# microsoft/fadtk

Measured on AMD Instinct MI355X. Metric: FAD scores/sec + cov-GEMM TFLOP/s (% MFMA peak), N=100k D=512, higher is better.
Workload: dtype f16 in, f16 MFMA with f32 accumulate over <= 8192-row runs, f64 across runs (moments); split-f16 MFMA iterations (f32 accumulate) + exact int8-MFMA products (int32 accumulate) + f64 correction (Frechet)

## Files before the change

fadtk_amd/csrc/frechet.hip:

```cpp
#include "frechet_internal.h"
#include "ns_mean.h"
#include "ns_fast.h"
#include "ns_fast_big.h"
#include "ns_fast_res.h"

#include <algorithm>
#include <atomic>
#include <cmath>
#include <type_traits>

namespace fad {

Pool& thread_pool(int device) {
    static thread_local PerThreadDevice<Pool> set;
    return set.get(device);
}
Workspace* free_slot(int device) {
    Pool& p = thread_pool(device);
    for (Workspace& w : p.slot)
        if (!w.busy) { w.pool = &p; return &w; }
    return nullptr;
}

SongKnobs SongKnobs::from_env() {
// ... 359 lines not shown
        g.k = k; g.max_low = max_low; g.nslots = nslots; g.chk_partials = m.partials;
        g.thr_pred = pred_threshold(ws.pool, d);
        fast_split(d, nsf::SP_U, g, stream, 1);
    }
    nsf::I8Args a;
    memset(&a, 0, sizeof(a));
    a.Adig = f.digY[0]; a.Bdig = f.digYt[0]; a.Adig_alt = f.digY[1]; a.Bdig_alt = f.digYt[1]; a.sel = &m.s32->final_iter;
    a.d = d; a.gen = ws.job.gen; a.hA = f.hdr; a.hB = f.hdr + 1; a.skip = &m.s32->skip_corr; a.stats = f.host_stats; a.st = m.dstate; a.A64in = m.A;
    a.Y[0] = f.Y[0]; a.Y[1] = f.Y[1]; a.Z[0] = f.Z[0]; a.Z[1] = f.Z[1];
    a.s32 = m.s32; a.host_words = f.host_words; a.host_vals = f.host_vals;
    const bool wide = wide_enabled(ws.pool);
    if (wide) { a.Rv = f.Rv; a.scaled = 1; }
    f.host_words[12] = 0;
    f.host_words[13] = 0;
    fast_i8(d, nsf::I8_G, a, stream);
    FAD_HIP_TRY(hipGetLastError());
    if (!ws.done_ev) FAD_HIP_TRY(hipEventCreateWithFlags(&ws.done_ev, hipEventDisableTiming));
    if (wide && ws.pool && ws.pool->lp_verify) return fast_verify_enqueue(ws);
    FAD_HIP_TRY(hipEventRecord(ws.done_ev, stream));
    return FAD_OK;
}

static void fast_decide_one(const int* hw, const double* hv, const double* hsx, int nb, MixedResult* out, const double* hvx = nullptr,
                            int gen = 0, int max_low = kMaxLow) {
    MixedResult o;
    memset(&o, 0, sizeof(o));
    const bool bad = hw[0] != 0;
    o.status = 0; o.iters = hw[7]; o.decided_at = hw[8]; o.nonfinite = hw[2]; o.too_few0 = hw[3]; o.too_few1 = hw[4];
    o.c = hv[0]; o.tr1 = hv[1]; o.tr2 = hv[2]; o.mean_term = hv[3];
    o.prepared = 0;
    const bool ok = hw[5] != 0, failed = hw[6] != 0, strict = hw[9] != 0;
    if (bad || hw[1] || failed) {
        o.status = 2;
    } else if (ok && !hw[11]) {
        double corr = 0.0, r2 = 0.0, tr = 0.0, zinf = 0.0, zone = 0.0;
        for (int t = 0; t < nb * nb; ++t) { corr += hsx[nsf::kTileStats * t]; r2 += hsx[nsf::kTileStats * t + 1]; tr += hsx[nsf::kTileStats * t + 2]; }
        const double* zmax = hsx + (size_t)nsf::kTileStats * nb * nb;
        for (int x = 0; x < nb; ++x) {
            double rs = 0.0, cs = 0.0;
            for (int y = 0; y < nb; ++y) { rs += zmax[2 * (y * nb + x)]; cs += zmax[2 * (x * nb + y) + 1]; }
            if (rs > zinf) zinf = rs;
            if (cs > zone) zone = cs;
        }
        const int fi = hw[7];
        double res = hv[4 + ns32_slot(fi)];
        if (hw[8] == fi - 1) { const double rp = hv[4 + ns32_slot(fi - 1)]; res = 0.75 * rp * rp + 0.25 * rp * rp * rp; if (res < 2e-6) res = 2e-6; }
        const double zn = std::sqrt(zinf * zone), rn = std::sqrt(r2);
        double trs = tr + 0.5 * corr;
        double est = zn * zn * zn * rn * rn / 8.0 + zn * res * rn / 2.0;
        bool finite = std::isfinite(trs) && std::isfinite(est);
        double fad = o.mean_term + o.tr1 + o.tr2 - 2.0 * std::sqrt(o.c) * trs;
        bool accept = finite && (est <= 1e-9 * std::fabs(trs) || 2.0 * std::sqrt(o.c) * est <= 1e-5 * std::fabs(fad));
        const bool scaled = hvx && hw[14] != 0;
        const bool predicted = hw[8] == fi - 1 && fi >= 1;
        const double r_pred = predicted ? hv[4 + ns32_slot(fi - 1)] : 0.0;
        const bool can_go_on = predicted && !strict && fi + 1 < max_low && (!scaled || r_pred > 0.1);
        bool need_verify = false;
        if (!accept && finite && hvx && !can_go_on) {
            if (hw[13] == gen) {
                const double inv = 1.0 / ((double)nsf::kVerScale * (double)nsf::kVerScale);
                double qp = 0.0, ep = 0.0, pp = 0.0, ee = 0.0;
// ... 34 lines not shown

bool fast_song_dim(int d) { return d == 128 || d == 256 || d == 384 || d == 512 || d == 768 || d == 1024; }

struct SongBlock {
    size_t hdr, st, s32, partials, stats, A64, P, Y[2], Z[2], T, digS, digY[2], digYt[2], stride;
};
static SongBlock song_block(int d) {
    const size_t dd = (size_t)d * d, nb = (size_t)d / 32;
    SongBlock b; size_t o = 0;
    auto take = [&](size_t bytes) { const size_t at = o; o += (bytes + 255) & ~(size_t)255; return at; };
    b.hdr = take(sizeof(nsf::MatHdr)); b.st = take(sizeof(NsState)); b.s32 = take(sizeof(Ns32State));
    b.partials = take(nb * nb * sizeof(double)); b.stats = take(nsf::kTileStats * nb * nb * sizeof(double));
    b.A64 = take(8 * dd); b.P = take(8 * dd);
    b.Y[0] = take(8 * dd); b.Y[1] = take(8 * dd); b.Z[0] = take(8 * dd); b.Z[1] = take(8 * dd); b.T = take(8 * dd);
    b.digS = take(6 * dd);
    b.digY[0] = take(6 * dd); b.digYt[0] = take(6 * dd); b.digY[1] = take(6 * dd); b.digYt[1] = take(6 * dd);
    b.stride = o;
    return b;
}
static size_t host_vstats_off(int d) {
    const size_t nb = (size_t)d / 32;
    return (nsf::kHostVals + (nsf::kTileStats + 2) * nb * nb) * sizeof(double) + ((nsf::kHostWords * sizeof(int) + 7) & ~(size_t)7);
}
static size_t song_host_stride(int d) {
    const size_t nb = (size_t)d / 32;
    return (host_vstats_off(d) + nsf::kVerStats * nb * nb * sizeof(double) + 63) & ~(size_t)63;
}
int64_t fast_songs_capacity(int d, size_t budget_bytes) {
    const int64_t n = (int64_t)(budget_bytes / song_block(d).stride);
    return n < 1 ? 1 : (n > 16384 ? 16384 : n);
}

int fast_songs(int d, int64_t B, const double* dcov_b, const double* covs, hipStream_t st, Workspace& ws,
               std::vector<double>& tr_sqrt, std::vector<char>& ok, int device, const SongKnobs& knobs) {
    const bool big = knobs.big_min > 0 && B >= knobs.big_min;
    const bool resident = d == 128 && knobs.res != 0;
    const bool res_full = resident && knobs.res != 1;
    const bool scaled_steps = knobs.scaled && big && d >= 256;
    const bool scaled_res = knobs.scaled && resident;
    const size_t dd = (size_t)d * d;
    const int nb = d / 32;
    const SongBlock L = song_block(d);
    const size_t hs = song_host_stride(d);
    FAD_TRY(ws.fast_songs.reserve(512 + 6 * dd + (size_t)B * L.stride));
    if (!ws.fast_songs_pin || ws.fast_songs_pin_cap < (size_t)B * hs) {
        if (ws.fast_songs_pin) (void)hipHostFree(ws.fast_songs_pin);
        ws.fast_songs_pin = nullptr; ws.fast_songs_pin_cap = 0;
        FAD_HIP_TRY(hipHostMalloc(&ws.fast_songs_pin, (size_t)B * hs + 4096, hipHostMallocDefault));
        ws.fast_songs_pin_cap = (size_t)B * hs + 4096;
    }
// ... 120 lines not shown
            if (hw[12] != gen) return set_error(FAD_ERR_HIP, "the correction kernel of the batched fast chain left no result for song %lld", (long long)b);
            MixedResult r;
            fast_decide_one(hw, hv, hx, nb, &r);
            if (r.status == 0 && k < kMaxLow && !resident) { pending = true; continue; }
            settled[b] = 1;
            if (r.status == 1) { ok[b] = 1; tr_sqrt[b] = std::sqrt(r.c) * r.tr_scaled; }
            if (trace)
                fprintf(stderr, "[fad fast songs] song %lld: status %d iters %d decided_at %d res %.3e est %.3e tr %.6e c %.3e (words bad %d done %d ok %d failed %d skipped %d)\n",
                        (long long)b, r.status, r.iters, r.decided_at, r.res, r.est, r.tr_scaled, r.c, hw[0], hw[1], hw[5], hw[6], hw[11]);
            if (trace && b == 0) {
                fprintf(stderr, "[fad fast songs] song 0 residuals:");
                for (int q = 1; q < 16 && q <= r.iters; ++q) fprintf(stderr, " %.3e", hv[4 + q]);
                fprintf(stderr, "\n");
            }
        }
        if (!pending) break;
        upto = kMaxLow;
    }
    return FAD_OK;
}


struct PairBlock {
    size_t hdrA, hdrB, st, s32, partials, stats, A64, P, Y[2], Z[2], T, digA, digB, digY[2], digYt[2], mus, covs, Rv, Pv, Ev, stride;
};
static PairBlock pair_block(int d) {
    const size_t dd = (size_t)d * d, nb = (size_t)d / 32;
    PairBlock b; size_t o = 0;
    auto take = [&](size_t bytes) { const size_t at = o; o += (bytes + 255) & ~(size_t)255; return at; };
    b.hdrA = take(sizeof(nsf::MatHdr)); b.hdrB = take(sizeof(nsf::MatHdr)); b.st = take(sizeof(NsState)); b.s32 = take(sizeof(Ns32State));
    b.partials = take(nb * nb * sizeof(double)); b.stats = take(nsf::kTileStats * nb * nb * sizeof(double));
    b.A64 = take(8 * dd); b.P = take(8 * dd);
    b.Y[0] = take(8 * dd); b.Y[1] = take(8 * dd); b.Z[0] = take(8 * dd); b.Z[1] = take(8 * dd); b.T = take(8 * dd);
    b.digA = take(6 * dd); b.digB = take(6 * dd);
    b.digY[0] = take(6 * dd); b.digYt[0] = take(6 * dd); b.digY[1] = take(6 * dd); b.digYt[1] = take(6 * dd);
    b.mus = take(2 * (size_t)d * sizeof(double)); b.covs = take(2 * dd * sizeof(double));
    b.Rv = take(8 * dd); b.Pv = take(8 * dd); b.Ev = take(8 * dd);
    b.stride = o;
    return b;
}

static int pairs_verify_enqueue(Workspace& ws, int d, int B, hipStream_t st) {
    const size_t dd = (size_t)d * d;
    const PairBlock L = pair_block(d);
    const size_t hs = song_host_stride(d);
    char* blk = static_cast<char*>(ws.fast_pairs.p);
    char* hpin = static_cast<char*>(ws.fast_pairs_pin);
    auto at = [&](size_t off) { return blk + off; };
    auto mat = [&](size_t off) { nsf::SplitMat m; m.a = reinterpret_cast<uint4*>(at(off)); m.at = reinterpret_cast<uint4*>(at(off + 4 * dd)); return m; };
    nsf::SplitArgs g;
    memset(&g, 0, sizeof(g));
    g.d = d; g.gen = ws.multi.gen; g.hA = reinterpret_cast<nsf::MatHdr*>(at(L.hdrA)); g.hB = reinterpret_cast<nsf::MatHdr*>(at(L.hdrB));
    g.pstride = (int64_t)L.stride; g.astride = (int64_t)L.stride;
    g.st = reinterpret_cast<NsState*>(at(L.st)); g.s32 = reinterpret_cast<Ns32State*>(at(L.s32));
    const nsf::SplitMat Y[2] = {mat(L.Y[0]), mat(L.Y[1])}, Z[2] = {mat(L.Z[0]), mat(L.Z[1])};
    const int nb = d / 32;
    int* h_words = reinterpret_cast<int*>(hpin + (nsf::kHostVals + (size_t)(nsf::kTileStats + 2) * nb * nb) * sizeof(double));
    double* h_vstats = reinterpret_cast<double*>(hpin + host_vstats_off(d));
    for (int b = 0; b < B; ++b) reinterpret_cast<int*>(reinterpret_cast<char*>(h_words) + (size_t)b * hs)[13] = 0;
    fast_verify_launch(d, (unsigned)B, g, Y, Z, mat(L.Rv), mat(L.Pv), mat(L.Ev), g.s32, h_vstats, h_words, (int64_t)hs, st);
    FAD_HIP_TRY(hipGetLastError());
    FAD_HIP_TRY(hipEventRecord(ws.done_ev, st));
    return FAD_OK;
}

static int pairs_enqueue(Workspace& ws, int d, int B, const fad_moments_t* const* h1, const fad_moments_t* const* h2, int ddof,
                         int mean_dtype, hipStream_t st) {
    const size_t dd = (size_t)d * d;
    const int nb = d / 32;
    constexpr int kPairsBigMin = 3;
    const bool big = B >= kPairsBigMin && d >= 256;
    const bool wide = wide_enabled(ws.pool);
    const int max_low = wide ? kMaxLowWide : kMaxLow;
    const int device = ws.job.device;
    const PairBlock L = pair_block(d);
    const size_t hs = song_host_stride(d);
    void* const before = ws.fast_pairs.p;
    FAD_TRY(ws.fast_pairs.reserve((size_t)(B > 16 ? kMaxMultiPairs : B > 8 ? 16 : B > 4 ? 8 : 4) * L.stride + 256));
    if (!ws.fast_pairs_pin || ws.fast_pairs_pin_cap < (size_t)B * hs) {
        if (ws.fast_pairs_pin) (void)hipHostFree(ws.fast_pairs_pin);
        ws.fast_pairs_pin = nullptr; ws.fast_pairs_pin_cap = 0;
        FAD_HIP_TRY(hipHostMalloc(&ws.fast_pairs_pin, (size_t)kMaxMultiPairs * hs + 4096, hipHostMallocDefault));
        ws.fast_pairs_pin_cap = (size_t)kMaxMultiPairs * hs + 4096;
    }
    char* blk = static_cast<char*>(ws.fast_pairs.p);
    char* hpin = static_cast<char*>(ws.fast_pairs_pin);
    double* h_vals = reinterpret_cast<double*>(hpin);
    double* h_stats = h_vals + nsf::kHostVals;
    int* h_words = reinterpret_cast<int*>(h_stats + (size_t)(nsf::kTileStats + 2) * nb * nb);
    auto at = [&](size_t off) { return blk + off; };
    auto mat = [&](size_t off) { nsf::SplitMat m; m.a = reinterpret_cast<uint4*>(at(off)); m.at = reinterpret_cast<uint4*>(at(off + 4 * dd)); return m; };
    const int gen = ++ws.fast_gen;
    if (ws.fast_gen > (1 << 30)) ws.fast_gen = 1;
    ws.multi.gen = gen;
// ... 21 lines not shown
    }
    pa.acc[0] = pa.accs[0]; pa.acc[1] = pa.accs[1];
    pa.d = d; pa.ddof = ddof; pa.gen = gen; pa.mean_dtype = mean_dtype;
    pa.mus = reinterpret_cast<double*>(at(L.mus)); pa.covs = reinterpret_cast<double*>(at(L.covs));
    pa.dig[0] = reinterpret_cast<uint4*>(at(L.digA)); pa.dig[1] = reinterpret_cast<uint4*>(at(L.digB));
    pa.st = st0; pa.hdr[0] = hA; pa.hdr[1] = hB;
    pa.batch = 2; pa.pstride = (int64_t)L.stride; pa.no_covs = 1;
    pa.per = ((dd / 2048) % 4 == 0) ? 4 : 2;
    hipLaunchKernelGGL(nsf::nsf_prepare, dim3((unsigned)(dd / 2048 / pa.per + 1), (unsigned)(2 * B)), dim3(512), 0, st, pa);

    auto split_args = [&]() {
        nsf::SplitArgs g;
        memset(&g, 0, sizeof(g));
        g.d = d; g.gen = gen; g.hA = hA; g.hB = hB; g.pstride = (int64_t)L.stride; g.astride = (int64_t)L.stride;
        g.st = st0; g.s32 = s32_0;
        if (wide) { g.scaled = 1; g.lp_wide = 1; g.l0_scale = kWideL0Scale; g.l0_min = kWideL0Min; }
        return g;
    };
    {
        nsf::I8Args a;
        memset(&a, 0, sizeof(a));
        a.Adig = reinterpret_cast<uint4*>(at(L.digA)); a.Bdig = reinterpret_cast<uint4*>(at(L.digB)); a.d = d; a.gen = gen; a.hA = hA; a.hB = hB;
        a.pstride = (int64_t)L.stride; a.astride = (int64_t)L.stride; a.stats = stats; a.A64 = A64; a.P = P; a.st = st0;
        if (big) FAD_TRY(fast_i8_big(d, nsf::I8_A, a, st, (unsigned)B, device));
        else fast_i8(d, nsf::I8_A, a, st, (unsigned)B);
        nsf::SplitArgs g = split_args();
        g.A[0] = P; g.B[0] = P; g.C[0] = Y[1]; g.C[1] = Z[1]; g.A64 = A64; g.statsA = stats;
        if (big) FAD_TRY(fast_split_big(d, nsf::SP_FIRST, g, st, (unsigned)B, device));
        else { g.Cdig[0] = digY[1]; g.Cdig_t[0] = digYt[1]; fast_split(d, nsf::SP_FIRST, g, st, (unsigned)B); }
    }
    int want = ws.pool ? ws.pool->lp_iters : 5;
    if (want < 2) want = 2;
    if (want > max_low) want = max_low;
    for (int k = 1; k < want; ++k) {
        const int cur = k & 1;
        nsf::SplitArgs g = split_args();
        g.A[0] = Z[cur]; g.B[0] = Y[cur]; g.C[0] = T; g.alpha = -0.5f; g.beta_eye = 1.5f; g.gamma = 1.0f;
        g.partials = partials; g.skip = &s32_0->done; g.k = k;
        if (big) FAD_TRY(fast_split_big(d, nsf::SP_T, g, st, (unsigned)B, device));
        else fast_split(d, nsf::SP_T, g, st, (unsigned)B);
        g = split_args();
        g.A[0] = Y[cur]; g.B[0] = T; g.C[0] = Y[cur ^ 1]; g.A[1] = T; g.B[1] = Z[cur]; g.C[1] = Z[cur ^ 1];
        if (!big) { g.Cdig[0] = digY[cur ^ 1]; g.Cdig_t[0] = digYt[cur ^ 1]; }
        g.skip = &s32_0->upd_skip[k & 1];
        g.k = k; g.max_low = max_low; g.nslots = big ? fast_big_t_slots(d, (unsigned)B) : nb * nb; g.chk_partials = partials; g.thr_pred = pred_threshold(ws.pool, d);
        if (big) FAD_TRY(fast_split_big(d, nsf::SP_U, g, st, (unsigned)B, device));
        else fast_split(d, nsf::SP_U, g, st, (unsigned)B);
    }
    if (big) {
        nsf::DigArgs dg;
        memset(&dg, 0, sizeof(dg));
        dg.d = d; dg.gen = gen; dg.hA = hA; dg.hB = hB; dg.pstride = (int64_t)L.stride; dg.astride = (int64_t)L.stride; dg.s32 = s32_0;
        dg.Y[0] = Y[0]; dg.Y[1] = Y[1]; dg.dig[0] = digY[0]; dg.dig[1] = digY[1]; dg.dig_t[0] = digYt[0]; dg.dig_t[1] = digYt[1];
        hipLaunchKernelGGL(nsf::nsf_digitize, dim3((unsigned)((dd / 16 + 255) / 256), 2, (unsigned)B), dim3(256), 0, st, dg);
    }
    {
        nsf::I8Args a;
        memset(&a, 0, sizeof(a));
        a.Adig = digY[0]; a.Bdig = digYt[0]; a.Adig_alt = digY[1]; a.Bdig_alt = digYt[1]; a.sel = &s32_0->final_iter;
        a.d = d; a.gen = gen; a.hA = hA; a.hB = hB; a.pstride = (int64_t)L.stride; a.astride = (int64_t)L.stride; a.hstride = (int64_t)hs;
        a.skip = &s32_0->skip_corr; a.stats = h_stats; a.st = st0; a.A64in = A64;
        a.Y[0] = Y[0]; a.Y[1] = Y[1]; a.Z[0] = Z[0]; a.Z[1] = Z[1]; a.s32 = s32_0; a.host_words = h_words; a.host_vals = h_vals;
        if (wide) { a.Rv = mat(L.Rv); a.scaled = 1; }
        for (int b = 0; b < B; ++b) { int* w = reinterpret_cast<int*>(reinterpret_cast<char*>(h_words) + (size_t)b * hs); w[12] = 0; w[13] = 0; }
        if (big) FAD_TRY(fast_i8_big(d, nsf::I8_G, a, st, (unsigned)B, device));
        else fast_i8(d, nsf::I8_G, a, st, (unsigned)B);
    }
    FAD_HIP_TRY(hipGetLastError());
    if (!ws.done_ev) FAD_HIP_TRY(hipEventCreateWithFlags(&ws.done_ev, hipEventDisableTiming));
    if (wide && ws.pool && ws.pool->lp_verify) return pairs_verify_enqueue(ws, d, B, st);
    FAD_HIP_TRY(hipEventRecord(ws.done_ev, st));
    return FAD_OK;
}

static int mixed_begin(const NsProblem& pb, int device, hipStream_t stream, Workspace& ws) {
    const int d = pb.d;
    const int64_t dd = (int64_t)d * d;
    FAD_TRY(ws.mats.reserve((size_t)(6 * dd) * sizeof(double)));
    FAD_TRY(ws.mats32.reserve((size_t)(5 * dd) * sizeof(float)));
    const size_t hbytes = ws.job.fast ? fast_pinned_bytes(d) : sizeof(NsState) + sizeof(MixedResult);
    if (!ws.pinned || ws.pinned_cap < hbytes) {
        if (ws.pinned) (void)hipHostFree(ws.pinned);
        ws.pinned = nullptr; ws.pinned_cap = 0;
        FAD_HIP_TRY(hipHostMalloc(&ws.pinned, hbytes + 4096, hipHostMallocDefault));
        ws.pinned_cap = hbytes + 4096;
    }
    MixedBufs m = mixed_bufs(ws, d);
    m.hres->status = -1;
    ws.job.d = d; ws.job.device = device; ws.job.stream = stream; ws.job.k = 0;
    if (ws.job.fast) {
        ws.job.mu1 = pb.mu1; ws.job.mu2 = pb.mu2; ws.job.mean_dtype = pb.mean_dtype;
        int want = ws.pool ? ws.pool->lp_iters : 5;
        if (want < 2) want = 2;
// ... 268 lines not shown
    *job = reinterpret_cast<fad_frechet_job_t*>(wsp);
    return FAD_OK;
}

int fad_frechet_multi_end(fad_frechet_job_t* job, int count, double* out_fad, fad_diag_t* diag) {
    if (!job || !out_fad) return set_error(FAD_ERR_INVALID, "NULL argument");
    Workspace& ws = *reinterpret_cast<Workspace*>(job);
    if (!ws.busy) return set_error(FAD_ERR_INVALID, "this job was collected already");
    if (count != ws.multi.count) return set_error(FAD_ERR_INVALID, "this job holds %d pairs, not %d", ws.multi.count, count);
    const Workspace::Job j = ws.job;
    const Workspace::Multi m = ws.multi;
    DeviceGuard g(j.device);
    const int d = j.d, nb = d / 32;
    bool done[kMaxMultiPairs] = {false};
    int chain_status[kMaxMultiPairs];
    for (int b = 0; b < kMaxMultiPairs; ++b) chain_status[b] = -1;
    int rc = FAD_OK;
    if (m.enqueued) {
        const hipError_t e = hipEventSynchronize(ws.done_ev);
        if (e != hipSuccess) { ws.busy = false; return set_error(FAD_ERR_HIP, "hipEventSynchronize failed: %s", hipGetErrorString(e)); }
        const size_t hs = song_host_stride(d);
        const char* hpin = static_cast<const char*>(ws.fast_pairs_pin);
        const size_t off_stats = nsf::kHostVals * sizeof(double), off_words = off_stats + (size_t)(nsf::kTileStats + 2) * nb * nb * sizeof(double);
        const size_t off_vstats = host_vstats_off(d);
        const bool wide = wide_enabled(ws.pool);
        int learnt = -1;
        bool any_verified = false;
        for (int round = 0; round < 2; ++round) {
            bool ask = false;
            for (int b = 0; b < count; ++b) {
                if (done[b]) continue;
                const double* hv = reinterpret_cast<const double*>(hpin + (size_t)b * hs);
                const double* hx = reinterpret_cast<const double*>(hpin + (size_t)b * hs + off_stats);
                const int* hw = reinterpret_cast<const int*>(hpin + (size_t)b * hs + off_words);
                const double* hvx = reinterpret_cast<const double*>(hpin + (size_t)b * hs + off_vstats);
                if (hw[12] != m.gen) continue;
                MixedResult r;
                fast_decide_one(hw, hv, hx, nb, &r, wide ? hvx : nullptr, m.gen, wide ? kMaxLowWide : kMaxLow);
                chain_status[b] = r.status;
                if (r.too_few0 || r.too_few1) {
                    if (rc == FAD_OK) rc = set_error(FAD_ERR_TOO_FEW_ROWS, "FAD requires at least two embedding window frames in each set");
                    out_fad[b] = NAN; done[b] = true;
                    continue;
                }
                if (r.status == 5 && round == 0) { ask = true; continue; }
                if (r.status != 1) continue;
                const double tr_sqrt = sqrt(r.c) * r.tr_scaled;
                out_fad[b] = r.mean_term + r.tr1 + r.tr2 - 2.0 * tr_sqrt;
                if (diag) {
                    fad_diag_t& q = diag[b];
                    memset(&q, 0, sizeof(q));
                    q.iters = r.iters + 1; q.converged = 3; q.used_eps = 0; q.route = 2;
                    q.residual = r.res; q.scale = r.c; q.mean_term = r.mean_term; q.tr1 = r.tr1; q.tr2 = r.tr2; q.tr_sqrt = tr_sqrt;
                    q.verified = r.pad == 1 ? 1 : 0;
                }
                if (r.decided_at + 1 > learnt) learnt = r.decided_at + 1;
                if (r.pad == 1) any_verified = true;
                done[b] = true;
            }
            if (!ask) break;
            const int rv = pairs_verify_enqueue(ws, d, count, j.stream);
            if (rv != FAD_OK) { if (rc == FAD_OK) rc = rv; break; }
            const hipError_t e2 = hipEventSynchronize(ws.done_ev);
            if (e2 != hipSuccess) { ws.busy = false; return set_error(FAD_ERR_HIP, "hipEventSynchronize failed: %s", hipGetErrorString(e2)); }
        }
        if (learnt > 0 && ws.pool) ws.pool->lp_iters = learnt;
        if (ws.pool && wide) ws.pool->lp_verify = any_verified;

        int declined = 0;
        for (int b = 0; b < count; ++b) if (!done[b] && chain_status[b] == 2) ++declined;
        if (rc == FAD_OK && declined >= 2) {
            const PairBlock L = pair_block(d);
            const size_t dd = (size_t)d * d;
            char* blk = static_cast<char*>(ws.fast_pairs.p);
            const int64_t stride = (int64_t)(L.stride / sizeof(double));
            const double* mus = reinterpret_cast<const double*>(blk + L.mus);
            const double* covs = reinterpret_cast<const double*>(blk + L.covs);
            int r2 = ws.small.reserve(ns_small_bytes(d, count));
            NsState* hst = nullptr;
            if (r2 == FAD_OK) {
                NsState* dstates = static_cast<NsState*>(ws.small.p);
                enqueue_clear_states(dstates, count, j.stream);
                uint32_t mask = 0;
                for (int b = 0; b < count; ++b) if (done[b] || chain_status[b] != 2) mask |= (1u << b);
// ... 56 lines not shown
```

fadtk_amd/csrc/frechet_internal.h:

```cpp
#pragma once
#include "fad_common.h"
#include "ns_check.h"
#include "ns32.h"

#include <cstdlib>
#include <vector>

struct fad_moments;
namespace fad {
const double* moments_packed(const fad_moments* h);
int moments_settle(const fad_moments* h, hipStream_t st);
int moments_mark_read(const fad_moments* h, hipStream_t st);
int moments_device(const fad_moments* h);
int moments_dim(const fad_moments* h);
const float* moments_runsum(const fad_moments* h);

constexpr int kStatScal = 8;
static inline int64_t stat_blocks(int d) { return cdiv(d, 32); }
static inline size_t stat_doubles(int d) { const int64_t nb = stat_blocks(d); return (size_t)(2 * nb * d + kStatScal * nb * nb); }

constexpr int kMaxMultiPairs = 32;

struct Workspace : NsWorkspace {
    DevBuf rows, offs, songbuf, songmat, rows2, songrun, songjobs;
    DevBuf base_root;
    void* song_pin = nullptr; size_t song_pin_cap = 0;
    DevBuf mats32;
    DevBuf fast;
    int fast_gen = 0;
    DevBuf songcov;
    DevBuf fast_songs;
    void* fast_songs_pin = nullptr; size_t fast_songs_pin_cap = 0;
    DevBuf fast_pairs;
    void* fast_pairs_pin = nullptr; size_t fast_pairs_pin_cap = 0;
    struct Multi {
        int count = 0, gen = 0;
        bool enqueued = false;
        const fad_moments_t* h1[kMaxMultiPairs] = {nullptr}; const fad_moments_t* h2[kMaxMultiPairs] = {nullptr};
    } multi;
    bool busy = false;
    struct Job {
        int d = 0, device = 0, k = 0, mean_dtype = -1, ddof = 1;
        bool mixed = false;
        bool fast = false;
        int gen = 0;
        double eps = 0.0;
        hipStream_t stream = nullptr;
        const double *cov1 = nullptr, *cov2 = nullptr, *mu1 = nullptr, *mu2 = nullptr;
    } job;
    hipEvent_t done_ev = nullptr;
    struct Pool* pool = nullptr;
    void release_all() {
        release(); rows.release(); offs.release(); songbuf.release(); songmat.release(); rows2.release(); songrun.release(); songjobs.release(); mats32.release(); base_root.release(); fast.release();
        fast_songs.release(); songcov.release(); fast_pairs.release();
        if (fast_pairs_pin) { (void)hipHostFree(fast_pairs_pin); fast_pairs_pin = nullptr; fast_pairs_pin_cap = 0; }
        if (fast_songs_pin) { (void)hipHostFree(fast_songs_pin); fast_songs_pin = nullptr; fast_songs_pin_cap = 0; }
        if (done_ev) { (void)hipEventDestroy(done_ev); done_ev = nullptr; }
        if (song_pin) { (void)hipHostFree(song_pin); song_pin = nullptr; song_pin_cap = 0; }
    }
    int reserve_song_pin(size_t bytes) {
// ... 87 lines not shown
```

fadtk_amd/csrc/ns_fast.h:

```cpp
#pragma once
#include "fad_common.h"
#include "ns_check.h"
#include "ns32.h"
#include "ns_mean.h"

namespace fad {
namespace nsf {

typedef int i32x4 __attribute__((ext_vector_type(4)));
typedef int i32x16 __attribute__((ext_vector_type(16)));
typedef _Float16 f16x8 __attribute__((ext_vector_type(8)));
typedef _Float16 f16x2 __attribute__((ext_vector_type(2)));

constexpr int kDigits = 6;
constexpr int kUminA = 3, kUminG = 4;
constexpr float kLoScale = 2048.f, kLoInv = 1.f / 2048.f;
constexpr int kTileStats = 4;

__device__ __host__ __forceinline__ size_t fa_idx(int rb, int ks, int plane, int lane, int d) {
    return (((size_t)rb * (size_t)(d >> 4) + (size_t)ks) * 2 + (size_t)plane) * 64 + (size_t)lane;
}
__device__ __host__ __forceinline__ size_t dg_idx(int rb, int ks, int p, int lane, int d) {
    return (((size_t)rb * (size_t)(d >> 5) + (size_t)ks) * kDigits + (size_t)p) * 64 + (size_t)lane;
}
// ... 270 lines not shown
}


enum { I8_A = 0, I8_G = 1 };
constexpr int kHostWords = 16, kHostVals = 24;
struct I8Args {
    const uint4* Adig; const uint4* Bdig;
    const uint4* Adig_alt; const uint4* Bdig_alt; const int* sel;
    int d, gen;
    const MatHdr* hA; const MatHdr* hB;
    int64_t pstride, hstride;
    int64_t astride;
    const int* skip;
    double* stats;
    double* A64; SplitMat P;
    NsState* st;
    const double* A64in;
    SplitMat Y[2], Z[2];
    const Ns32State* s32;
    int* host_words;
    double* host_vals;
    SplitMat Rv;
    int scaled;
};
constexpr float kVerScale = 4096.f;
constexpr int kVerStats = 4;

template <int NS8, int MODE>
__global__ __launch_bounds__(512) void nsf_i8(I8Args g) {
    __shared__ __attribute__((aligned(16))) double part[2 * 32 * 33];
    __shared__ float fin[32 * 33];
    __shared__ float finR[(MODE == I8_G) ? 32 * 33 : 1];
    __shared__ double red[8 * 4];
    constexpr int kUmin = (MODE == I8_A) ? kUminA : kUminG;
    constexpr int kGroups = 2 * (kDigits - 1) - kUmin + 1;
    const int d = g.d, tid = threadIdx.x, lane = tid & 63;
    const int64_t po = (int64_t)blockIdx.z * g.pstride, ho = (int64_t)blockIdx.z * g.hstride;
    const MatHdr* hB = adv(g.hB, po);
    const MatHdr* hA = adv(g.hA, (int64_t)blockIdx.z * g.astride);
    NsState* const st_p = adv(g.st, po);
    const bool bad = hdr_bad(hA, hB, g.gen);
    const bool skipped = bad || (g.skip && *adv(g.skip, po) != 0);
    if constexpr (MODE == I8_G) {
        if (blockIdx.x == 0 && blockIdx.y == 0 && tid == 0) {
            const NsState* st = st_p; const Ns32State* s = adv(g.s32, po);
            int* hw = adv(g.host_words, ho); double* hv = adv(g.host_vals, ho);
            hw[0] = bad ? 1 : 0; hw[1] = st->done; hw[2] = st->nonfinite; hw[3] = st->too_few[0]; hw[4] = st->too_few[1];
// ... 450 lines not shown
```

fadtk_amd/csrc/ns_fast_big.h:

```cpp
#pragma once
#include "ns_fast.h"
#include "big_slots.h"

namespace fad {
namespace nsf {

#ifndef FAD_BIG_STAGES
#define FAD_BIG_STAGES 3
#endif
constexpr int kBigStages = FAD_BIG_STAGES;
constexpr int kBigStage = 1024;
constexpr size_t kBigLds = (size_t)kBigStages * kBigStage * 16 + 256;

template <int MODE, int NJ = 2>
__global__ __launch_bounds__(256, (FAD_BIG_STAGES <= 3) ? 3 : ((FAD_BIG_STAGES <= 4) ? 2 : 1)) void nsf_big(SplitArgs g) {
    static_assert(MODE == SP_T || MODE == SP_U || MODE == SP_FIRST, "SP_FIRST: iteration 0 (scale from nsf_i8<A>'s statistics, Y1, Z1)");
    extern __shared__ __attribute__((aligned(16))) uint4 ring[];
    double* red = reinterpret_cast<double*>(ring + kBigStages * kBigStage);
    const int d = g.d, tid = threadIdx.x, lane = tid & 63;
    constexpr int ZP = (MODE == SP_U) ? 2 : 1;
    const int t = d >> 7, tx_n = (NJ == 2) ? t : 2 * t, tt = t * tx_n;
    const int L = blockIdx.x;
    const int nprod = big_grid(g.nprob, tt * ZP);
    if constexpr (MODE == SP_U) {
// ... 206 lines not shown
            __builtin_amdgcn_wave_barrier();
#pragma unroll
            for (int pass = 0; pass < 4; ++pass) store_tile_planes(fin, Cm, by, bx, d, pass * 64 + lane);
            if (with_digits) {
#pragma unroll 2
                for (int pass = 0; pass < 8; ++pass) store_tile_digits(fin, dig, dig_t, by, bx, d, pass * 64 + lane);
            }
            __builtin_amdgcn_wave_barrier();
        }
    if constexpr (MODE == SP_T) {
        double s1[1] = {ss};
        wg8_sum<1, 4>(s1, red);
        if (tid == 0) adv(g.partials, po)[tile] = s1[0];
    }
}

constexpr int kI8BigStage = 36 * 64;
#ifndef FAD_I8_BIG_STAGES
#define FAD_I8_BIG_STAGES 2
#endif
constexpr int kI8BigStages = FAD_I8_BIG_STAGES;
constexpr size_t kI8BigLds = (size_t)kI8BigStages * kI8BigStage * 16 + 256;

template <int MODE, bool WITHR = false>
__global__ __launch_bounds__(512) void nsf_i8_big(I8Args g, int nprob) {
    extern __shared__ __attribute__((aligned(16))) uint4 ring[];
    double* red = reinterpret_cast<double*>(ring + kI8BigStages * kI8BigStage);
    constexpr int kUmin = (MODE == I8_A) ? kUminA : kUminG;
    constexpr int kGroups = 2 * (kDigits - 1) - kUmin + 1;
    const int d = g.d, tid = threadIdx.x, lane = tid & 63;
    const int tr_ = d >> 7, tc_ = d >> 6, tt = tr_ * tc_;
    const BigSlot slot = big_slot(blockIdx.x, nprob, tt);
    if (!slot.live) return;
    const int song = slot.song, tile = slot.item;
    const int TY = tile / tc_, TX = tile - TY * tc_;
    const int64_t po = (int64_t)song * g.pstride, ho = (int64_t)song * g.hstride;
    const MatHdr* hB = adv(g.hB, po);
    const MatHdr* hA = adv(g.hA, (int64_t)song * g.astride);
    NsState* const st_p = adv(g.st, po);
    const bool bad = hdr_bad(hA, hB, g.gen);
    const bool skipped = bad || (g.skip && *adv(g.skip, po) != 0);
    if constexpr (MODE == I8_G) {
        if (tile == 0 && tid == 0) {
            const NsState* st = st_p; const Ns32State* s = adv(g.s32, po);
            int* hw = adv(g.host_words, ho); double* hv = adv(g.host_vals, ho);
            hw[0] = bad ? 1 : 0; hw[1] = st->done; hw[2] = st->nonfinite; hw[3] = st->too_few[0]; hw[4] = st->too_few[1];
            hw[5] = s->ok; hw[6] = s->failed; hw[7] = s->final_iter; hw[8] = s->decided_at; hw[9] = s->strict; hw[10] = s->finished;
            hw[11] = skipped ? 1 : 0;
            hv[0] = st->c; hv[1] = st->tr1; hv[2] = st->tr2; hv[3] = st->mean_term;
#pragma unroll
            for (int q = 0; q < 16; ++q) hv[4 + q] = s->res[q];
            hw[14] = (g.scaled && st->mu[0] != 1.0) ? 1 : 0;
            hw[12] = g.gen;
        }
    }
    if (skipped) return;
    const int wave = __builtin_amdgcn_readfirstlane(tid >> 6);
    const int wr = wave >> 1, wc = wave & 1;
    const bool alt = (MODE == I8_G) && g.sel && (*adv(g.sel, po) & 1);
    const uint4* Ad = (MODE == I8_A) ? adv(g.Adig, (int64_t)song * g.astride) : adv(alt ? g.Adig_alt : g.Adig, po);
    const uint4* Bd = adv(alt ? g.Bdig_alt : g.Bdig, po);
#ifdef FAD_I8_ABL_G_NOLOOP
    const int nks = (MODE == I8_G) ? 0 : (d >> 5);
#else
    const int nks = d >> 5;
#endif

    const uint32_t voff = (uint32_t)lane * 16u;
    const uint32_t ring_lds = (uint32_t)(size_t)(__attribute__((address_space(3))) void*)ring;
    auto issue = [&](int ks) {
#pragma unroll
        for (int i = 0; i < 5; ++i) {
            const int q = wave + 8 * i;
            if (q < 36) {
                const bool bs = q >= 24;
                const int blk = bs ? (q - 24) / 6 : q / 6, p = bs ? (q - 24) % 6 : q % 6;
                const uint64_t sb = (uint64_t)((bs ? Bd : Ad) + dg_idx((bs ? 2 * TX : 4 * TY) + blk, ks, p, 0, d));
                const uint32_t lo = __builtin_amdgcn_readfirstlane((uint32_t)sb);
// ... 30 lines not shown
        for (int p = 0; p < kDigits; ++p) { acc[0][p] += a[p][0] ^ b[p][1]; acc[1][p] += a[p][2] ^ b[p][3]; }
#else
#pragma unroll
        for (int p = kDigits - 1; p >= 0; --p)
#pragma unroll
            for (int q = kDigits - 1; q >= 0; --q)
                if (p + q >= kUmin) acc[p + q - kUmin] = __builtin_amdgcn_mfma_i32_32x32x32_i8(a[p], b[q], acc[p + q - kUmin], 0, 0, 0);
#endif
    }
    __syncthreads();
    double gp[16];
#pragma unroll
    for (int q = 0; q < 16; ++q) gp[q] = 0.0;
#pragma unroll
    for (int u = 0; u < kGroups; ++u) {
        const double wgt = __builtin_ldexp(1.0, 7 * (u + kUmin) - 80);
#pragma unroll
        for (int q = 0; q < 16; ++q) gp[q] = __builtin_fma((double)acc[u][q], wgt, gp[q]);
    }
    float* fin = reinterpret_cast<float*>(ring) + wave * (32 * 33 + 32);
    const int kg = lane >> 5, n = lane & 31;
    const int by = 4 * TY + wr, bx = 2 * TX + wc, nb = d >> 5;
    const int row0 = 32 * by, col0 = 32 * bx;
    double* const stats = adv(g.stats, (MODE == I8_A) ? po : ho);
    double* scal = stats + (size_t)kTileStats * (by * nb + bx);
    double v3[3] = {0.0, 0.0, 0.0};
    if constexpr (MODE == I8_A) {
        const double inv = hdr_inv_s12(hA, hB);
        double* A64 = adv(g.A64, po) + (int64_t)(row0 + 4 * kg) * d + col0 + n;
#pragma unroll
        for (int reg = 0; reg < 16; ++reg) {
            const int q = (reg & 3) + 8 * (reg >> 2);
            A64[(int64_t)q * d] = gp[reg] * inv;
            fin[(q + 4 * kg) * 33 + n] = (float)gp[reg];
            v3[0] += gp[reg] * gp[reg];
            if (by == bx && q + 4 * kg == n) v3[1] += gp[reg];
        }
        __builtin_amdgcn_wave_barrier();
        const SplitMat Pm = adv(g.P, po);
#pragma unroll
        for (int pass = 0; pass < 4; ++pass) store_tile_planes(fin, Pm, by, bx, d, pass * 64 + lane);
    } else {
        const SplitMat Zm = adv(g.Z[alt ? 1 : 0], po);
        const SplitMat Ym = adv(g.Y[alt ? 1 : 0], po);
        const double inv_c = 1.0 / st_p->c;
        const double* A64 = adv(g.A64in, po) + (int64_t)(row0 + 4 * kg) * d + col0 + n;
        typedef _Float16 f16x4 __attribute__((ext_vector_type(4)));
// ... 20 lines not shown
            fin[(q + 4 * kg) * 33 + n] = fabsf((float)z);
        }
        __builtin_amdgcn_wave_barrier();
    }
    double m = 0.0;
    if constexpr (MODE == I8_A) {
        if (lane < 32) { for (int c = 0; c < 32; ++c) m += fabsf(fin[lane * 33 + c]); }
        else { for (int q = 0; q < 32; ++q) m += fabsf(fin[q * 33 + lane - 32]); }
    } else {
        if (lane < 32) { for (int q = 0; q < 32; ++q) m += fin[q * 33 + lane]; }
        else { for (int c = 0; c < 32; ++c) m += fin[(lane - 32) * 33 + c]; }
    }
    double mrow = (lane < 32) ? m : 0.0, mcol = (lane >= 32) ? m : 0.0;
#pragma unroll
    for (int off = 32; off > 0; off >>= 1) {
        mrow = fmax(mrow, __shfl_xor(mrow, off)); mcol = fmax(mcol, __shfl_xor(mcol, off));
#pragma unroll
        for (int q = 0; q < 3; ++q) v3[q] += __shfl_xor(v3[q], off);
    }
    if (lane == 0) {
        if constexpr (MODE == I8_A) {
            scal[0] = v3[0]; scal[1] = v3[1]; scal[2] = mrow; scal[3] = mcol;
        } else {
            scal[0] = v3[0]; scal[1] = v3[1]; scal[2] = v3[2]; scal[3] = 0.0;
            double* zmax = stats + (size_t)kTileStats * nb * nb + 2 * (size_t)(by * nb + bx);
            zmax[0] = mrow; zmax[1] = mcol;
        }
    }
    if constexpr (MODE == I8_G && WITHR) {
        if (g.Rv.a) {
            __builtin_amdgcn_wave_barrier();
#pragma unroll
            for (int reg = 0; reg < 16; ++reg) fin[((reg & 3) + 8 * (reg >> 2) + 4 * kg) * 33 + n] = (float)(gp[reg] * (double)kVerScale);
            __builtin_amdgcn_wave_barrier();
            const SplitMat Rm = adv(g.Rv, po);
#pragma unroll
            for (int pass = 0; pass < 4; ++pass) store_tile_planes(fin, Rm, by, bx, d, pass * 64 + lane);
        }
    }
    (void)red;
}

}
}
```

Before: 12790.

## Reduce per-tile correction stats on device via last-block ticket in big pairs path

In the big multi-pair I8_G correction kernel, each tile writes its stats to a device-side record with atomic stores. The last-arriving block, found through an atomic counter, reduces them into five totals that go to pinned host memory, so the host decision no longer walks nb*nb tile stats per pair. The R-verification matrix write is also deferred: it is produced only when verification is actually requested, by relaunching the correction kernel with R enabled. This adds an arrival counter, a fence protocol and an extra kernel launch on the verify path.

```diff
diff --git a/fadtk_amd/csrc/frechet.hip b/fadtk_amd/csrc/frechet.hip
--- a/fadtk_amd/csrc/frechet.hip
+++ b/fadtk_amd/csrc/frechet.hip
@@ -405,7 +405,7 @@
 }
 
 static void fast_decide_one(const int* hw, const double* hv, const double* hsx, int nb, MixedResult* out, const double* hvx = nullptr,
-                            int gen = 0, int max_low = kMaxLow) {
+                            int gen = 0, int max_low = kMaxLow, const double* tot = nullptr) {
     MixedResult o;
     memset(&o, 0, sizeof(o));
     const bool bad = hw[0] != 0;
@@ -417,9 +417,10 @@
         o.status = 2;
     } else if (ok && !hw[11]) {
         double corr = 0.0, r2 = 0.0, tr = 0.0, zinf = 0.0, zone = 0.0;
-        for (int t = 0; t < nb * nb; ++t) { corr += hsx[nsf::kTileStats * t]; r2 += hsx[nsf::kTileStats * t + 1]; tr += hsx[nsf::kTileStats * t + 2]; }
+        if (tot) { corr = tot[0]; r2 = tot[1]; tr = tot[2]; zinf = tot[3]; zone = tot[4]; }
+        else for (int t = 0; t < nb * nb; ++t) { corr += hsx[nsf::kTileStats * t]; r2 += hsx[nsf::kTileStats * t + 1]; tr += hsx[nsf::kTileStats * t + 2]; }
         const double* zmax = hsx + (size_t)nsf::kTileStats * nb * nb;
-        for (int x = 0; x < nb; ++x) {
+        for (int x = 0; x < nb && !tot; ++x) {
             double rs = 0.0, cs = 0.0;
             for (int y = 0; y < nb; ++y) { rs += zmax[2 * (y * nb + x)]; cs += zmax[2 * (x * nb + y) + 1]; }
             if (rs > zinf) zinf = rs;
@@ -500,10 +501,11 @@
     const size_t nb = (size_t)d / 32;
     return (nsf::kHostVals + (nsf::kTileStats + 2) * nb * nb) * sizeof(double) + ((nsf::kHostWords * sizeof(int) + 7) & ~(size_t)7);
 }
-static size_t song_host_stride(int d) {
+static size_t host_totals_off(int d) {
     const size_t nb = (size_t)d / 32;
-    return (host_vstats_off(d) + nsf::kVerStats * nb * nb * sizeof(double) + 63) & ~(size_t)63;
-}
+    return host_vstats_off(d) + nsf::kVerStats * nb * nb * sizeof(double);
+}
+static size_t song_host_stride(int d) { return (host_totals_off(d) + nsf::kHostTotals * sizeof(double) + 63) & ~(size_t)63; }
 int64_t fast_songs_capacity(int d, size_t budget_bytes) {
     const int64_t n = (int64_t)(budget_bytes / song_block(d).stride);
     return n < 1 ? 1 : (n > 16384 ? 16384 : n);
@@ -670,7 +672,7 @@
 
 
 struct PairBlock {
-    size_t hdrA, hdrB, st, s32, partials, stats, A64, P, Y[2], Z[2], T, digA, digB, digY[2], digYt[2], mus, covs, Rv, Pv, Ev, stride;
+    size_t hdrA, hdrB, st, s32, partials, stats, A64, P, Y[2], Z[2], T, digA, digB, digY[2], digYt[2], mus, covs, Rv, Pv, Ev, tilerec, arrive, stride;
 };
 static PairBlock pair_block(int d) {
     const size_t dd = (size_t)d * d, nb = (size_t)d / 32;
@@ -684,6 +686,7 @@
     b.digY[0] = take(6 * dd); b.digYt[0] = take(6 * dd); b.digY[1] = take(6 * dd); b.digYt[1] = take(6 * dd);
     b.mus = take(2 * (size_t)d * sizeof(double)); b.covs = take(2 * dd * sizeof(double));
     b.Rv = take(8 * dd); b.Pv = take(8 * dd); b.Ev = take(8 * dd);
+    b.tilerec = take((nsf::kTileStats + 2) * nb * nb * sizeof(double)); b.arrive = take(sizeof(unsigned));
     b.stride = o;
     return b;
 }
@@ -712,12 +715,46 @@
     return FAD_OK;
 }
 
+constexpr int kPairsBigMin = 3;
+static bool pairs_big(int d, int B) { return B >= kPairsBigMin && d >= 256; }
+
+static int pairs_correction_launch(Workspace& ws, int d, int B, bool with_r, hipStream_t st) {
+    const size_t dd = (size_t)d * d;
+    const int nb = d / 32;
+    const PairBlock L = pair_block(d);
+    const size_t hs = song_host_stride(d);
+    char* blk = static_cast<char*>(ws.fast_pairs.p);
+    char* hpin = static_cast<char*>(ws.fast_pairs_pin);
+    double* h_vals = reinterpret_cast<double*>(hpin);
+    double* h_stats = h_vals + nsf::kHostVals;
+    int* h_words = reinterpret_cast<int*>(h_stats + (size_t)(nsf::kTileStats + 2) * nb * nb);
+    auto at = [&](size_t off) { return blk + off; };
+    auto mat = [&](size_t off) { nsf::SplitMat m; m.a = reinterpret_cast<uint4*>(at(off)); m.at = reinterpret_cast<uint4*>(at(off + 4 * dd)); return m; };
+    const Ns32State* s32_0 = reinterpret_cast<const Ns32State*>(at(L.s32));
+    nsf::I8Args a;
+    memset(&a, 0, sizeof(a));
+    a.Adig = reinterpret_cast<uint4*>(at(L.digY[0])); a.Bdig = reinterpret_cast<uint4*>(at(L.digYt[0]));
+    a.Adig_alt = reinterpret_cast<uint4*>(at(L.digY[1])); a.Bdig_alt = reinterpret_cast<uint4*>(at(L.digYt[1])); a.sel = &s32_0->final_iter;
+    a.d = d; a.gen = ws.multi.gen; a.hA = reinterpret_cast<nsf::MatHdr*>(at(L.hdrA)); a.hB = reinterpret_cast<nsf::MatHdr*>(at(L.hdrB));
+    a.pstride = (int64_t)L.stride; a.astride = (int64_t)L.stride; a.hstride = (int64_t)hs;
+    a.skip = &s32_0->skip_corr; a.stats = h_stats; a.st = reinterpret_cast<NsState*>(at(L.st)); a.A64in = reinterpret_cast<const double*>(at(L.A64));
+    a.Y[0] = mat(L.Y[0]); a.Y[1] = mat(L.Y[1]); a.Z[0] = mat(L.Z[0]); a.Z[1] = mat(L.Z[1]); a.s32 = s32_0; a.host_words = h_words; a.host_vals = h_vals;
+    if (wide_enabled(ws.pool)) a.scaled = 1;
+    if (with_r) a.Rv = mat(L.Rv);
+    if (pairs_big(d, B)) {
+        a.tile_rec = reinterpret_cast<double*>(at(L.tilerec)); a.arrive = reinterpret_cast<unsigned*>(at(L.arrive));
+        a.totals = reinterpret_cast<double*>(hpin + host_totals_off(d));
+        return fast_i8_big(d, nsf::I8_G, a, st, (unsigned)B, ws.job.device);
+    }
+    fast_i8(d, nsf::I8_G, a, st, (unsigned)B);
+    return FAD_OK;
+}
+
 static int pairs_enqueue(Workspace& ws, int d, int B, const fad_moments_t* const* h1, const fad_moments_t* const* h2, int ddof,
                          int mean_dtype, hipStream_t st) {
     const size_t dd = (size_t)d * d;
     const int nb = d / 32;
-    constexpr int kPairsBigMin = 3;
-    const bool big = B >= kPairsBigMin && d >= 256;
+    const bool big = pairs_big(d, B);
     const bool wide = wide_enabled(ws.pool);
     const int max_low = wide ? kMaxLowWide : kMaxLow;
     const int device = ws.job.device;
@@ -785,8 +822,10 @@
         memset(&a, 0, sizeof(a));
         a.Adig = reinterpret_cast<uint4*>(at(L.digA)); a.Bdig = reinterpret_cast<uint4*>(at(L.digB)); a.d = d; a.gen = gen; a.hA = hA; a.hB = hB;
         a.pstride = (int64_t)L.stride; a.astride = (int64_t)L.stride; a.stats = stats; a.A64 = A64; a.P = P; a.st = st0;
-        if (big) FAD_TRY(fast_i8_big(d, nsf::I8_A, a, st, (unsigned)B, device));
-        else fast_i8(d, nsf::I8_A, a, st, (unsigned)B);
+        if (big) {
+            a.arrive = reinterpret_cast<unsigned*>(at(L.arrive));
+            FAD_TRY(fast_i8_big(d, nsf::I8_A, a, st, (unsigned)B, device));
+        } else fast_i8(d, nsf::I8_A, a, st, (unsigned)B);
         nsf::SplitArgs g = split_args();
         g.A[0] = P; g.B[0] = P; g.C[0] = Y[1]; g.C[1] = Z[1]; g.A64 = A64; g.statsA = stats;
         if (big) FAD_TRY(fast_split_big(d, nsf::SP_FIRST, g, st, (unsigned)B, device));
@@ -817,21 +856,14 @@
         dg.Y[0] = Y[0]; dg.Y[1] = Y[1]; dg.dig[0] = digY[0]; dg.dig[1] = digY[1]; dg.dig_t[0] = digYt[0]; dg.dig_t[1] = digYt[1];
         hipLaunchKernelGGL(nsf::nsf_digitize, dim3((unsigned)((dd / 16 + 255) / 256), 2, (unsigned)B), dim3(256), 0, st, dg);
     }
-    {
-        nsf::I8Args a;
-        memset(&a, 0, sizeof(a));
-        a.Adig = digY[0]; a.Bdig = digYt[0]; a.Adig_alt = digY[1]; a.Bdig_alt = digYt[1]; a.sel = &s32_0->final_iter;
-        a.d = d; a.gen = gen; a.hA = hA; a.hB = hB; a.pstride = (int64_t)L.stride; a.astride = (int64_t)L.stride; a.hstride = (int64_t)hs;
-        a.skip = &s32_0->skip_corr; a.stats = h_stats; a.st = st0; a.A64in = A64;
-        a.Y[0] = Y[0]; a.Y[1] = Y[1]; a.Z[0] = Z[0]; a.Z[1] = Z[1]; a.s32 = s32_0; a.host_words = h_words; a.host_vals = h_vals;
-        if (wide) { a.Rv = mat(L.Rv); a.scaled = 1; }
-        for (int b = 0; b < B; ++b) { int* w = reinterpret_cast<int*>(reinterpret_cast<char*>(h_words) + (size_t)b * hs); w[12] = 0; w[13] = 0; }
-        if (big) FAD_TRY(fast_i8_big(d, nsf::I8_G, a, st, (unsigned)B, device));
-        else fast_i8(d, nsf::I8_G, a, st, (unsigned)B);
-    }
+    const bool verify = wide && ws.pool && ws.pool->lp_verify;
+    for (int b = 0; b < B; ++b) { int* w = reinterpret_cast<int*>(reinterpret_cast<char*>(h_words) + (size_t)b * hs); w[12] = 0; w[13] = 0; }
+    ws.multi.with_r = verify;
+    ws.multi.totals = big;
+    FAD_TRY(pairs_correction_launch(ws, d, B, verify, st));
     FAD_HIP_TRY(hipGetLastError());
     if (!ws.done_ev) FAD_HIP_TRY(hipEventCreateWithFlags(&ws.done_ev, hipEventDisableTiming));
-    if (wide && ws.pool && ws.pool->lp_verify) return pairs_verify_enqueue(ws, d, B, st);
+    if (verify) return pairs_verify_enqueue(ws, d, B, st);
     FAD_HIP_TRY(hipEventRecord(ws.done_ev, st));
     return FAD_OK;
 }
@@ -1146,7 +1178,7 @@
         const size_t hs = song_host_stride(d);
         const char* hpin = static_cast<const char*>(ws.fast_pairs_pin);
         const size_t off_stats = nsf::kHostVals * sizeof(double), off_words = off_stats + (size_t)(nsf::kTileStats + 2) * nb * nb * sizeof(double);
-        const size_t off_vstats = host_vstats_off(d);
+        const size_t off_vstats = host_vstats_off(d), off_totals = host_totals_off(d);
         const bool wide = wide_enabled(ws.pool);
         int learnt = -1;
         bool any_verified = false;
@@ -1160,7 +1192,8 @@
                 const double* hvx = reinterpret_cast<const double*>(hpin + (size_t)b * hs + off_vstats);
                 if (hw[12] != m.gen) continue;
                 MixedResult r;
-                fast_decide_one(hw, hv, hx, nb, &r, wide ? hvx : nullptr, m.gen, wide ? kMaxLowWide : kMaxLow);
+                const double* tot = m.totals ? reinterpret_cast<const double*>(hpin + (size_t)b * hs + off_totals) : nullptr;
+                fast_decide_one(hw, hv, hx, nb, &r, wide ? hvx : nullptr, m.gen, wide ? kMaxLowWide : kMaxLow, tot);
                 chain_status[b] = r.status;
                 if (r.too_few0 || r.too_few1) {
                     if (rc == FAD_OK) rc = set_error(FAD_ERR_TOO_FEW_ROWS, "FAD requires at least two embedding window frames in each set");
@@ -1183,7 +1216,8 @@
                 done[b] = true;
             }
             if (!ask) break;
-            const int rv = pairs_verify_enqueue(ws, d, count, j.stream);
+            int rv = m.with_r ? FAD_OK : pairs_correction_launch(ws, d, count, true, j.stream);
+            if (rv == FAD_OK) rv = pairs_verify_enqueue(ws, d, count, j.stream);
             if (rv != FAD_OK) { if (rc == FAD_OK) rc = rv; break; }
             const hipError_t e2 = hipEventSynchronize(ws.done_ev);
             if (e2 != hipSuccess) { ws.busy = false; return set_error(FAD_ERR_HIP, "hipEventSynchronize failed: %s", hipGetErrorString(e2)); }
diff --git a/fadtk_amd/csrc/frechet_internal.h b/fadtk_amd/csrc/frechet_internal.h
--- a/fadtk_amd/csrc/frechet_internal.h
+++ b/fadtk_amd/csrc/frechet_internal.h
@@ -36,6 +36,8 @@
     struct Multi {
         int count = 0, gen = 0;
         bool enqueued = false;
+        bool with_r = false;
+        bool totals = false;
         const fad_moments_t* h1[kMaxMultiPairs] = {nullptr}; const fad_moments_t* h2[kMaxMultiPairs] = {nullptr};
     } multi;
     bool busy = false;
diff --git a/fadtk_amd/csrc/ns_fast.h b/fadtk_amd/csrc/ns_fast.h
--- a/fadtk_amd/csrc/ns_fast.h
+++ b/fadtk_amd/csrc/ns_fast.h
@@ -316,7 +316,11 @@
     double* host_vals;
     SplitMat Rv;
     int scaled;
+    double* tile_rec;
+    unsigned* arrive;
+    double* totals;
 };
+constexpr int kHostTotals = 5;
 constexpr float kVerScale = 4096.f;
 constexpr int kVerStats = 4;
 
diff --git a/fadtk_amd/csrc/ns_fast_big.h b/fadtk_amd/csrc/ns_fast_big.h
--- a/fadtk_amd/csrc/ns_fast_big.h
+++ b/fadtk_amd/csrc/ns_fast_big.h
@@ -252,6 +252,47 @@
 constexpr int kI8BigStages = FAD_I8_BIG_STAGES;
 constexpr size_t kI8BigLds = (size_t)kI8BigStages * kI8BigStage * 16 + 256;
 
+__device__ __forceinline__ void rec_put(double* p, double v) {
+    __hip_atomic_store(reinterpret_cast<unsigned long long*>(p), (unsigned long long)__double_as_longlong(v), __ATOMIC_RELAXED, __HIP_MEMORY_SCOPE_AGENT);
+}
+__device__ __forceinline__ double rec_get(const double* p) {
+    return __longlong_as_double((long long)__hip_atomic_load(reinterpret_cast<const unsigned long long*>(p), __ATOMIC_RELAXED, __HIP_MEMORY_SCOPE_AGENT));
+}
+__device__ __forceinline__ void i8_big_totals(const double* rec, int nb, double* out, double* sc, int tid) {
+    const int n = nb * nb;
+    double* const lrec = sc + 128;
+    for (int i = tid; i < (kTileStats + 2) * n; i += 512) lrec[i] = rec_get(rec + i);
+    __syncthreads();
+    if (tid < 3) {
+        double s = 0.0;
+        int t = 0;
+        for (; t + 8 <= n; t += 8) {
+            double v[8];
+#pragma unroll
+            for (int q = 0; q < 8; ++q) v[q] = lrec[kTileStats * (t + q) + tid];
+#pragma unroll
+            for (int q = 0; q < 8; ++q) s += v[q];
+        }
+        for (; t < n; ++t) s += lrec[kTileStats * t + tid];
+        sc[64 + tid] = s;
+    } else if (tid >= 64 && tid < 128) {
+        const double* zmax = lrec + (size_t)kTileStats * n;
+        const int x = tid & 31; const bool col = tid >= 96;
+        double s = 0.0;
+        if (x < nb) for (int y = 0; y < nb; ++y) s += col ? zmax[2 * (x * nb + y) + 1] : zmax[2 * (y * nb + x)];
+        sc[tid - 64] = s;
+    }
+    __syncthreads();
+    if (tid == 0) {
+        double zinf = 0.0, zone = 0.0;
+        for (int x = 0; x < nb; ++x) {
+            if (sc[x] > zinf) zinf = sc[x];
+            if (sc[32 + x] > zone) zone = sc[32 + x];
+        }
+        out[0] = sc[64]; out[1] = sc[65]; out[2] = sc[66]; out[3] = zinf; out[4] = zone;
+    }
+}
+
 template <int MODE, bool WITHR = false>
 __global__ __launch_bounds__(512) void nsf_i8_big(I8Args g, int nprob) {
     extern __shared__ __attribute__((aligned(16))) uint4 ring[];
@@ -284,6 +325,9 @@
             hw[12] = g.gen;
         }
     }
+    if constexpr (MODE == I8_A) {
+        if (g.arrive && tile == 0 && tid == 0) *adv(g.arrive, po) = 0u;
+    }
     if (skipped) return;
     const int wave = __builtin_amdgcn_readfirstlane(tid >> 6);
     const int wr = wave >> 1, wc = wave & 1;
@@ -360,7 +404,8 @@
     const int kg = lane >> 5, n = lane & 31;
     const int by = 4 * TY + wr, bx = 2 * TX + wc, nb = d >> 5;
     const int row0 = 32 * by, col0 = 32 * bx;
-    double* const stats = adv(g.stats, (MODE == I8_A) ? po : ho);
+    const bool own_totals = (MODE == I8_G) && g.totals;
+    double* const stats = own_totals ? adv(g.tile_rec, po) : adv(g.stats, (MODE == I8_A) ? po : ho);
     double* scal = stats + (size_t)kTileStats * (by * nb + bx);
     double v3[3] = {0.0, 0.0, 0.0};
     if constexpr (MODE == I8_A) {
@@ -427,9 +472,14 @@
         if constexpr (MODE == I8_A) {
             scal[0] = v3[0]; scal[1] = v3[1]; scal[2] = mrow; scal[3] = mcol;
         } else {
-            scal[0] = v3[0]; scal[1] = v3[1]; scal[2] = v3[2]; scal[3] = 0.0;
             double* zmax = stats + (size_t)kTileStats * nb * nb + 2 * (size_t)(by * nb + bx);
-            zmax[0] = mrow; zmax[1] = mcol;
+            if (own_totals) {
+                rec_put(scal, v3[0]); rec_put(scal + 1, v3[1]); rec_put(scal + 2, v3[2]); rec_put(scal + 3, 0.0);
+                rec_put(zmax, mrow); rec_put(zmax + 1, mcol);
+            } else {
+                scal[0] = v3[0]; scal[1] = v3[1]; scal[2] = v3[2]; scal[3] = 0.0;
+                zmax[0] = mrow; zmax[1] = mcol;
+            }
         }
     }
     if constexpr (MODE == I8_G && WITHR) {
@@ -443,6 +493,26 @@
             for (int pass = 0; pass < 4; ++pass) store_tile_planes(fin, Rm, by, bx, d, pass * 64 + lane);
         }
     }
+    if constexpr (MODE == I8_G) {
+        if (own_totals) {
+            asm volatile("s_waitcnt vmcnt(0)" ::: "memory");
+            __syncthreads();
+            unsigned* const ticket = reinterpret_cast<unsigned*>(red);
+            unsigned* const cnt = adv(g.arrive, po);
+            if (tid == 0) {
+                const unsigned before = __hip_atomic_fetch_add(cnt, 1u, __ATOMIC_RELAXED, __HIP_MEMORY_SCOPE_AGENT);
+                if (before == (unsigned)tt - 1u) {
+                    __builtin_amdgcn_fence(__ATOMIC_ACQUIRE, "agent");
+                    asm volatile("s_waitcnt vmcnt(0)" ::: "memory");
+                }
+                *ticket = before;
+            }
+            __syncthreads();
+            if (*ticket != (unsigned)tt - 1u) return;
+            i8_big_totals(stats, nb, adv(g.totals, ho), reinterpret_cast<double*>(ring), tid);
+            if (tid == 0) __hip_atomic_store(cnt, 0u, __ATOMIC_RELAXED, __HIP_MEMORY_SCOPE_AGENT);
+        }
+    }
     (void)red;
 }
 
```

Result: slower. 12520 (-2.1%).
